# heracles-ec/heracles

Hardware: AMD Instinct MI355X
Metric: map->Cl pairs/sec + mixing-matrix build sec, nside=4096 lmax=6144 (higher is better)
Workload: dtype f64

## Files before the change

heracles_amd/csrc/hx_ring_fft.hip:

```cpp
#include <algorithm>
#include <type_traits>

#include "hx_sht_common.h"


namespace hx {
__global__ __launch_bounds__(512) void k_init_bhat(PlanDev P, const int *__restrict__ rp_list,
                                                   double2 *__restrict__ bhat)
{
    extern __shared__ double2 buf[];
    const int rp = rp_list[blockIdx.x];
    const int n = P.nsub[rp];
    const int M = fft_size_for(n);
    for (int j = threadIdx.x; j < lds_fft_slots(M); j += blockDim.x) buf[j] = make_double2(0.0, 0.0);
    __syncthreads();
    for (int j = threadIdx.x; j < n; j += blockDim.x) {
        double2 c = expipi((double)chirp_num(j, n) / (double)n);
        buf[lds_slot(j)] = c;
        if (j) buf[lds_slot(M - j)] = c;
    }
    __syncthreads();
    lds_fft_dif(buf, M, P.tw, P.twN);
    double2 *out = bhat + P.bhat_off[rp];
    for (int e = threadIdx.x; e < M; e += blockDim.x) out[M >= 16 ? (e & 15) * (M >> 4) + (e >> 4) : e] = buf[lds_slot(e)];
}

__host__ __device__ inline int ring_ph_hi(int M) { return (4 * M) / 64 + 1; }
constexpr int RING_NTMAX = 512;
constexpr int RING_FB = 8;

template <int MODE, bool WSYM = false>
__global__ __launch_bounds__(RING_NTMAX) void k_ring_subdft(PlanDev P, const RingDesc *__restrict__ desc, int nrings, int nb, int Mclass,
                                                            const double *__restrict__ maps,
                                                            const double *__restrict__ pixw,
                                                            const double2 *__restrict__ zin,
                                                            double2 *__restrict__ Y, double *__restrict__ pixout = nullptr,
                                                            const double *__restrict__ ref = nullptr)
{
    extern __shared__ double2 buf[];
    __shared__ double2 tw_hi[TW_HI_MAX], tw_lo[64];
    double2 *ph_hi = buf + lds_fft_slots(Mclass), *ph_lo = ph_hi + ring_ph_hi(Mclass);
    const int nt = blockDim.x;
    const int nitems = ((nrings + 7) >> 3) * nb * 32;
    const TwFactored twf = load_tw_factored(tw_hi, tw_lo, P.tw, P.twN);
    int tid = threadIdx.x;
    auto ring_of = [&](int item) __attribute__((always_inline)) { return ((item >> 5) / nb) * 8 + (item & 7); };
    RingDesc cur = RingDesc{0, 0, 0, 1, 0};
    if ((int)blockIdx.x < nitems && ring_of(blockIdx.x) < nrings) cur = desc[ring_of(blockIdx.x)];
    for (int item = blockIdx.x; item < nitems; item += gridDim.x) {
        const int r = (item >> 3) & 3, set = item >> 5;
        const int ring = ring_of(item), c = set % nb;
        const int itn = item + gridDim.x, ringn = itn < nitems ? ring_of(itn) : nrings;
        const bool nextv = ringn < nrings;
        if (ring >= nrings) {
            if (nextv) cur = desc[ringn];
            continue;
        }
        const int n = cur.n;
        const long long sN = cur.sN, sS = cur.sS;
        const int M = fft_size_for(n), MP = lds_fft_slots(M);
        const bool blu = M != n;
        const int p = ilog2(M);
        const double2 *bh = P.bhat + cur.bhat_off;
        const double inv = 1.0 / M, inv4n = 0.25 / (double)n;
        asm volatile("; item" : "+v"(tid));
        const bool haveS = sS >= 0, odd = r & 1, pw = MODE == 0 && !WSYM && pixw != nullptr;
        constexpr bool wsym = MODE == 0 && WSYM;
        const double sg = (r & 2) ? -1.0 : 1.0;
        const double *mpN = maps + (long long)c * P.npix + sN, *mpS = maps + (long long)c * P.npix + (haveS ? sS : sN);
        const double *pwN = pixw + sN, *pwS = pixw + (haveS ? sS : sN);
        const double2 *zp = zin + (long long)c * P.ny + sN;
        double2 z[RING_FB][4];
        struct __attribute__((aligned(8))) Pair { double x, y; };
        Pair wsy[RING_FB / 2];
        auto load_batch_t = [&](auto WIDEC, int u0) __attribute__((always_inline)) {
            constexpr bool WIDE = decltype(WIDEC)::value;
#pragma unroll
            for (int u = 0; u < RING_FB; u += 2) {
                const int j = 2 * (tid + ((u0 + u) >> 1) * nt);
                const bool tail = WIDE && j == n - 1;
                const int jj = tail ? n - 2 : (j + 1 < n ? j : 0);
                wsy[u >> 1] = Pair{1.0, 1.0};
                if (MODE == 0 && wsym && WIDE) wsy[u >> 1] = *reinterpret_cast<const Pair *>(pwN + jj);
#pragma unroll
                for (int q = 0; q < 4; ++q) {
                    const int i = jj + q * n;
                    if (MODE == 0) {
                        Pair fn, fs;
                        if (WIDE) {
                            fn = *reinterpret_cast<const Pair *>(mpN + i);
                            fs = *reinterpret_cast<const Pair *>(mpS + i);
                            if (!wsym && pw) {
                                const Pair wn = *reinterpret_cast<const Pair *>(pwN + i), ws = *reinterpret_cast<const Pair *>(pwS + i);
                                fn.x *= wn.x; fn.y *= wn.y; fs.x *= ws.x; fs.y *= ws.y;
                            }
// ... 16 lines not shown
        auto load_batch = [&](int u0) __attribute__((always_inline)) {
            if (n >= 2) load_batch_t(std::true_type{}, u0);
            else load_batch_t(std::false_type{}, u0);
        };
        auto finish_batch = [&](int u0) __attribute__((always_inline)) {
            if (MODE != 0 || n < 2) return;
#pragma unroll
            for (int u = 0; u < RING_FB; u += 2) {
                const int j = 2 * (tid + ((u0 + u) >> 1) * nt);
                const bool tail = j == n - 1;
                const Pair w = wsy[u >> 1];
#pragma unroll
                for (int q = 0; q < 4; ++q) {
                    const double2 rn = z[u][q], rs = z[u + 1][q];
                    const double nx = wsym ? rn.x * w.x : rn.x, ny = wsym ? rn.y * w.y : rn.y;
                    const double sx = wsym ? rs.x * w.x : rs.x, sy = wsym ? rs.y * w.y : rs.y;
                    z[u][q] = make_double2(tail ? ny : nx, haveS ? (tail ? sy : sx) : 0.0);
                    z[u + 1][q] = make_double2(ny, haveS ? sy : 0.0);
                }
            }
        };
        load_batch(0);
        int4 nd0 = make_int4(0, 0, 0, 0), nd1 = nd0;
        if (nextv) {
            const int4 *dp = reinterpret_cast<const int4 *>(desc + ringn) + (tid >> 30);
            nd0 = dp[0];
            nd1 = dp[1];
        }
        auto lds_barrier = []() __attribute__((always_inline)) {
            __builtin_amdgcn_s_waitcnt(0xc07f);
            __builtin_amdgcn_s_barrier();
        };
        lds_barrier();
        for (int a = tid; a <= (4 * n) >> 6; a += nt) ph_hi[a] = expipi(-(double)(a << 6) / (2.0 * n));
        if (tid < 64) ph_lo[tid] = expipi(-(double)tid / (2.0 * n));
        lds_barrier();
        auto phase = [&](unsigned q) __attribute__((always_inline)) {
            return cmul(ph_hi[q >> 6], ph_lo[q & 63]);
        };
        {
            for (int u0 = 0;;) {
                finish_batch(u0);
#pragma unroll
                for (int u = 0; u < RING_FB; ++u) {
                    const int j = 2 * (tid + ((u0 + u) >> 1) * nt) + (u & 1);
                    const double2 e0 = odd ? csub(z[u][0], z[u][2]) : cadd(z[u][0], z[u][2]);
                    const double2 e1 = odd ? mul_mi(csub(z[u][1], z[u][3])) : cadd(z[u][1], z[u][3]);
                    const double2 t = make_double2(fma(sg, e1.x, e0.x), fma(sg, e1.y, e0.y));
                    const unsigned jc = j < n ? j : 0;
                    const unsigned qn = blu ? mod_by_inv(jc * (unsigned)r + 2u * jc * jc, 4u * (unsigned)n, inv4n) : jc * (unsigned)r;
                    buf[j < n ? lds_slot(j) : MP - 1] = cmul(t, phase(qn));
                }
                u0 += RING_FB;
                if (u0 * nt >= n) break;
                load_batch(u0);
            }
            if (blu)
                for (int j = n + tid; j < M; j += nt) buf[lds_slot(j)] = make_double2(0.0, 0.0);
        }
        __syncthreads();
        if (nextv) {
            auto sc = [](int v) __attribute__((always_inline)) { return __builtin_amdgcn_readfirstlane(v); };
            cur.sN = ((long long)sc(nd0.y) << 32) | (unsigned)sc(nd0.x);
            cur.sS = ((long long)sc(nd0.w) << 32) | (unsigned)sc(nd0.z);
            cur.bhat_off = ((long long)sc(nd1.y) << 32) | (unsigned)sc(nd1.x);
            cur.n = sc(nd1.z);
            cur.rp = sc(nd1.w);
        }
        double2 *out = Y + (long long)c * P.ny + sN + (long long)r * n;
        double *pxN = nullptr, *pxS = nullptr;
        const double *rfN = nullptr, *rfS = nullptr;
        if (MODE == 1 && pixout) {
            pxN = pixout + (long long)c * P.npix + sN + r;
            pxS = pixout + (long long)c * P.npix + (haveS ? sS : sN) + r;
            if (ref) { rfN = ref + (long long)c * P.npix + sN + r; rfS = ref + (long long)c * P.npix + (haveS ? sS : sN) + r; }
        }
        const int kdrop0 = MODE == 0 ? (P.lmax - r) / 4 + 1 : n, kdrop1 = (4 * n - P.lmax - r + 3) / 4;
        auto emit = [&](int k, double2 v) __attribute__((always_inline)) {
            if (MODE == 0 && k >= kdrop0 && k < kdrop1) return;
            if (MODE == 1 && pxN) {
                double fn = v.x, fs = -v.y;
                if (rfN) { fn = rfN[4 * k] - fn; fs = rfS[4 * k] - fs; }
                pxN[4 * k] = fn;
                if (haveS) pxS[4 * k] = fs;
            } else {
                out[k] = v;
            }
        };
        if (!blu) {
            lds_fft_dif(buf, M, twf, P.twN);
            for (int k = tid; k < n; k += nt) emit(k, buf[lds_slot(bitrev(k, p))]);
            continue;
        }
        if (M >= 16) {
            double2 bq[16];
            const int nbf = M >> 4;
#pragma unroll
            for (int j = 0; j < 16; ++j) bq[j] = bh[j * nbf + (tid < nbf ? tid : 0)];
            lds_fft_dif(buf, M, twf, P.twN, tid, nt, true);
#pragma unroll 1
            for (int i = tid; i < nbf; i += nt) {
                double2 x[16];
#pragma unroll
                for (int j = 0; j < 16; ++j) x[j] = buf[lds_slot(16 * i) + j];
                dif_regs<4>(x);
#pragma unroll
                for (int j = 0; j < 16; ++j) {
                    x[j] = cmul(x[j], bq[j]);
                }
                if (i + nt < nbf) {
#pragma unroll
                    for (int j = 0; j < 16; ++j) bq[j] = bh[j * nbf + i + nt];
                }
                dit_inv_regs<4>(x);
#pragma unroll
                for (int j = 0; j < 16; ++j) buf[lds_slot(16 * i) + j] = x[j];
            }
            __syncthreads();
            lds_fft_dit_inv(buf, M, twf, P.twN, tid, nt, true);
        } else {
            lds_fft_dif(buf, M, twf, P.twN, tid, nt);
            for (int j = tid; j < M; j += nt) buf[lds_slot(j)] = cmul(buf[lds_slot(j)], bh[j]);
            __syncthreads();
            lds_fft_dit_inv(buf, M, twf, P.twN, tid, nt);
        }
        for (int k = tid; k < n; k += nt)
            emit(k, cscale(cmul(buf[lds_slot(k)], phase(2u * mod_by_inv((unsigned)k * (unsigned)k, 2u * (unsigned)n, 2.0 * inv4n))), inv));
    }
}

template <int MODE, bool WSYM = false>
__global__ __launch_bounds__(RING_NTMAX) void k_ring_pairfft(PlanDev P, const RingDesc *__restrict__ desc, int nrings, int nb, int M,
                                                             const double *__restrict__ maps, const double *__restrict__ pixw,
                                                             const double2 *__restrict__ zin, double2 *__restrict__ Y,
                                                             double *__restrict__ pixout = nullptr, const double *__restrict__ ref = nullptr)
{
    extern __shared__ double2 buf[];
    __shared__ double2 tw_hi[TW_HI_MAX], tw_lo[64];
    const int MP = lds_fft_slots(M), n = M, p = ilog2(M);
    double2 *ph_hi = buf + 2 * MP, *ph_lo = ph_hi + ring_ph_hi(M);
    const int nt = blockDim.x, nh = nt >> 1;
    const int nitems = ((nrings + 7) >> 3) * nb * 16;
    const TwFactored twf = load_tw_factored(tw_hi, tw_lo, P.tw, P.twN);
    int tid = threadIdx.x;
    for (int a = tid; a <= (4 * n) >> 6; a += nt) ph_hi[a] = expipi(-(double)(a << 6) / (2.0 * n));
    if (tid < 64) ph_lo[tid] = expipi(-(double)tid / (2.0 * n));
    __syncthreads();
    auto phase = [&](unsigned q) __attribute__((always_inline)) { return cmul(ph_hi[q >> 6], ph_lo[q & 63]); };
    auto ring_of = [&](int item) __attribute__((always_inline)) { return ((item >> 4) / nb) * 8 + (item & 7); };
    auto comp_of = [&](int item) __attribute__((always_inline)) { return (item >> 4) % nb; };
    RingDesc cur = RingDesc{0, 0, 0, 1, 0};
    if ((int)blockIdx.x < nitems && ring_of(blockIdx.x) < nrings) cur = desc[ring_of(blockIdx.x)];
    struct __attribute__((aligned(8))) Pair { double x, y; };
    double2 z[RING_FB][4];
    Pair wsy[RING_FB / 2];
    const bool pw = MODE == 0 && !WSYM && pixw != nullptr;
    constexpr bool wsym = MODE == 0 && WSYM;
    auto request = [&](auto U0C, const RingDesc &d, int c) __attribute__((always_inline)) {
        constexpr int U0 = decltype(U0C)::value;
        const bool hS = d.sS >= 0;
// ... 80 lines not shown
            request(H0{}, cur, comp_of(itn));
            have_half = true;
        }
        const int half = tid >= nh ? 1 : 0, gt = tid - half * nh;
        double2 *bh = buf + half * MP;
        lds_fft_dif(bh, M, twf, P.twN, gt, nh);
        const int r = rpair + 2 * half;
        if (MODE == 1 && pixout) {
            double *pxN = pixout + (long long)c * P.npix + sN + r, *pxS = pixout + (long long)c * P.npix + (haveS ? sS : sN) + r;
            if (ref) {
                const double *rfN = ref + (long long)c * P.npix + sN + r, *rfS = ref + (long long)c * P.npix + (haveS ? sS : sN) + r;
                for (int k = gt; k < n; k += nh) {
                    const double2 v = bh[lds_slot(bitrev(k, p))];
                    pxN[4 * k] = rfN[4 * k] - v.x;
                    if (haveS) pxS[4 * k] = rfS[4 * k] + v.y;
                }
            } else {
                for (int k = gt; k < n; k += nh) {
                    const double2 v = bh[lds_slot(bitrev(k, p))];
                    pxN[4 * k] = v.x;
                    if (haveS) pxS[4 * k] = -v.y;
                }
            }
        } else {
            double2 *out = Y + (long long)c * P.ny + sN + (long long)r * n;
            const int kdrop0 = MODE == 0 ? (P.lmax - r) / 4 + 1 : n, kdrop1 = (4 * n - P.lmax - r + 3) / 4;
            for (int k = gt; k < n; k += nh)
                if (k < kdrop0 || k >= kdrop1) *(out + k) = bh[lds_slot(bitrev(k, p))];
        }
        }
    }
}

constexpr int SPLIT_JMAX = 16;

__global__ __launch_bounds__(512) void k_init_bhat_split(PlanDev P, const int *__restrict__ rp_list, int C,
                                                          double2 *__restrict__ bhat)
{
    extern __shared__ double2 buf[];
    const int rp = rp_list[blockIdx.x];
    const int n = P.nsub[rp], M = 2 * C;
    double2 *out = bhat + P.bhat_off[rp];
    auto b_at = [&](int j) {
        const int jj = j < n ? j : (M - j < n ? M - j : -1);
        return jj < 0 ? make_double2(0.0, 0.0) : expipi((double)chirp_num(jj, n) / (double)n);
    };
    for (int half = 0; half < 2; ++half) {
        __syncthreads();
        for (int j = threadIdx.x; j < C; j += blockDim.x) {
            const double2 b0 = b_at(j), b1 = b_at(j + C);
            buf[lds_slot(j)] = half == 0 ? cadd(b0, b1) : cmul(csub(b0, b1), P.tw[j]);
        }
        __syncthreads();
        lds_fft_dif(buf, C, P.tw, P.twN);
        for (int j = threadIdx.x; j < C; j += blockDim.x) out[half * C + j] = buf[lds_slot(j)];
    }
}

template <int MODE>
__global__ __launch_bounds__(512) void k_ring_subdft_split(PlanDev P, const int *__restrict__ rp_list, int C,
                                                            const double *__restrict__ maps, const double *__restrict__ pixw,
                                                            const double2 *__restrict__ zin, double2 *__restrict__ Y,
                                                            double *__restrict__ pixout = nullptr, const double *__restrict__ ref = nullptr)
{
    extern __shared__ double2 buf[];
    const int rp = rp_list[blockIdx.y];
// ... 94 lines not shown
__global__ __launch_bounds__(256) void k_pixw_symmetry(PlanDev P, const double *__restrict__ pixw, int *__restrict__ flag)
{
    const int rp = blockIdx.x, n = P.nsub[rp];
    const long long sN = P.startN[rp], sS = P.startS[rp];
    bool ok = true;
    for (int j = threadIdx.x; j < n; j += blockDim.x) {
        const double w = pixw[sN + j];
#pragma unroll
        for (int q = 1; q < 4; ++q) ok = ok && pixw[sN + j + (long long)q * n] == w;
        if (sS >= 0) {
#pragma unroll
            for (int q = 0; q < 4; ++q) ok = ok && pixw[sS + j + (long long)q * n] == w;
        }
    }
    if (!ok) *flag = 0;
}

}

using namespace hx;

static int g_lds_fft_cap = 8192;
extern "C" int hx_set_max_lds_fft(int points)
{
    if (points < 16 || points > 8192 || (points & (points - 1))) return fail(HX_ERR_ARG, "hx_set_max_lds_fft: a power of two in [16, 8192]");
    g_lds_fft_cap = points;
    return HX_OK;
}

static size_t ring_class_lds(int M, bool pair) { return ((pair ? 2 : 1) * (size_t)lds_fft_slots(M) + ring_ph_hi(M) + 64) * sizeof(double2); }

static bool ring_class_is_pair(int n, int M, int cap) { return M == n && M >= 16 && M <= cap && ring_class_lds(M, true) + 4096 <= 160 * 1024; }

int hx::ring_fft_plan_init(hx_plan *pl, const std::vector<int> &nsub, const std::vector<long long> &sN, const std::vector<long long> &sS)
{
    const int cap = g_lds_fft_cap;
    std::map<std::pair<int, int>, std::vector<int>> byM;
    bool plain_beyond_cap = false;
    for (int rp = pl->nrp - 1; rp >= 0; --rp) {
        const int M = fft_size_for(nsub[rp]);
        byM[{M, ring_class_is_pair(nsub[rp], M, cap) ? -1 : 0}].push_back(rp);
        plain_beyond_cap = plain_beyond_cap || (M > cap && M == nsub[rp]);
    }
    const int maxM = byM.rbegin()->first.first;
    if (maxM > 2 * cap || plain_beyond_cap) return fail(HX_ERR_UNSUPPORTED, "hx_plan_create: nside=%d needs an in-LDS FFT of %d points (limit %d, %d for Bluestein rings); unsupported", pl->nside, maxM, cap, 2 * cap);
    pl->fft_cap = cap;
    pl->lds_fft = (size_t)lds_fft_slots(std::min(maxM, cap)) * sizeof(double2);
    for (auto it = byM.rbegin(); it != byM.rend(); ++it) {
        pl->fft_classes.push_back({it->first.first, (int)pl->h_fft_rp_list.size(), (int)it->second.size(), it->first.second});
        pl->h_fft_rp_list.insert(pl->h_fft_rp_list.end(), it->second.begin(), it->second.end());
    }
    HX_TRY(upload(pl->fft_rp_list, pl->h_fft_rp_list));
    std::vector<long long> boff(pl->nrp, -1);
    std::vector<int> blu_list, blu_split;
    long long btot = 0;
    std::map<int, long long> off_of_n;
    for (int rp = 0; rp < pl->nrp; ++rp) {
        int n = nsub[rp], M = fft_size_for(n);
        if (M == n) continue;
        auto it = off_of_n.find(n);
        if (it == off_of_n.end()) {
            it = off_of_n.emplace(n, btot).first;
            btot += M;
            (M > cap ? blu_split : blu_list).push_back(rp);
        }
        boff[rp] = it->second;
    }
    HX_TRY(upload(pl->bhat_off, boff));
    std::vector<RingDesc> desc;
    for (int rp : pl->h_fft_rp_list) desc.push_back(RingDesc{sN[rp], sS[rp], boff[rp], nsub[rp], rp});
    HX_TRY(upload(pl->fft_desc, desc));
    HX_TRY(pl->bhat.alloc(sizeof(double2) * std::max<long long>(btot, 1)));
    const void *const init_kernels[] = {(const void *)k_init_bhat, (const void *)k_init_bhat_split};
    const void *const ring_kernels[] = {(const void *)k_ring_subdft<0, false>,  (const void *)k_ring_subdft<0, true>,  (const void *)k_ring_subdft<1, false>,
                                        (const void *)k_ring_pairfft<0, false>, (const void *)k_ring_pairfft<0, true>, (const void *)k_ring_pairfft<1, false>,
                                        (const void *)k_ring_subdft_split<0>,   (const void *)k_ring_subdft_split<1>};
    for (const void *k : init_kernels) (void)hipFuncSetAttribute(k, hipFuncAttributeMaxDynamicSharedMemorySize, 160 * 1024);
    for (const void *k : ring_kernels) (void)hipFuncSetAttribute(k, hipFuncAttributeMaxDynamicSharedMemorySize, 156 * 1024);
    HX_HIP(hipGetLastError());
    hipStream_t st = rt().stream;
    if (!blu_list.empty()) {
        DevBuf d_list;
        HX_TRY(upload(d_list, blu_list));
        hipLaunchKernelGGL(k_init_bhat, dim3((unsigned)blu_list.size()), dim3(512), pl->lds_fft, st, pl->dev(),
                           d_list.as<int>(), pl->bhat.as<double2>());
        (void)hipStreamSynchronize(st);
    }
    if (!blu_split.empty()) {
        DevBuf d_list;
        HX_TRY(upload(d_list, blu_split));
        hipLaunchKernelGGL(k_init_bhat_split, dim3((unsigned)blu_split.size()), dim3(std::min(512, std::max(64, cap / 16))), (size_t)lds_fft_slots(cap) * sizeof(double2), st,
                           pl->dev(), d_list.as<int>(), cap, pl->bhat.as<double2>());
        (void)hipStreamSynchronize(st);
    }
    return HX_OK;
}

struct RingIO { const double *maps, *pixw; const double2 *zin; double2 *Y; double *pixout; const double *ref; };

template <auto KERNEL>
static void launch_ring_class(hx_plan *pl, const hx_plan::FftClass &c, int nb, const RingIO &io)
{
    const int k = c.big < 0 ? 2 : 1;
    const int threads = std::min(RING_NTMAX, k * std::max(64, c.M / 16));
    const size_t lds = ring_class_lds(c.M, k == 2);
    const int per_cu = (int)std::max<size_t>(1, std::min<size_t>(512 / threads, (160 * 1024) / (lds + 3 * 1024 + 256)));
    const long long items = ((long long)c.count + 7) / 8 * nb * (32 / k);
    const unsigned groups = (unsigned)std::min<long long>(items, (long long)rt().cus * per_cu);
    hipLaunchKernelGGL(KERNEL, dim3(groups), dim3(threads), lds, rt().stream, pl->dev(), pl->fft_desc.as<RingDesc>() + c.first, c.count, nb, c.M, io.maps, io.pixw, io.zin, io.Y, io.pixout, io.ref);
}

template <int MODE, bool WSYM>
static int launch_subdft_classes(hx_plan *pl, int nb, const RingIO &io, int rp_lo = 0, int rp_hi = 0x7fffffff)
{
    for (const auto &cls : pl->fft_classes) {
        hx_plan::FftClass c = cls;
        if (rp_lo > 0 || rp_hi < pl->nrp) {
            const int *b = pl->h_fft_rp_list.data() + cls.first, *e = b + cls.count;
            const int *x = std::lower_bound(b, e, rp_hi, [](int rp, int lim) { return rp >= lim; });
            const int *y = std::lower_bound(b, e, rp_lo, [](int rp, int lim) { return rp >= lim; });
            c.first = cls.first + (int)(x - b);
            c.count = (int)(y - x);
            if (c.count <= 0) continue;
        }
        if (c.big < 0)
            launch_ring_class<k_ring_pairfft<MODE, WSYM>>(pl, c, nb, io);
        else if (c.M > pl->fft_cap) {
            const int C = pl->fft_cap, threads = std::min(512, std::max(64, C / SPLIT_JMAX));
            hipLaunchKernelGGL(k_ring_subdft_split<MODE>, dim3(1, c.count, nb), dim3(threads), (size_t)lds_fft_slots(C) * sizeof(double2), rt().stream,
                               pl->dev(), pl->fft_rp_list.as<int>() + c.first, C, io.maps, io.pixw, io.zin, io.Y, io.pixout, io.ref);
        } else
            launch_ring_class<k_ring_subdft<MODE, WSYM>>(pl, c, nb, io);
    }
    HX_HIP(hipGetLastError());
    return HX_OK;
}

int hx::launch_ring_subdft_maps(hx_plan *pl, int nb, const double *d_maps, const double *d_pw, double2 *Y, int rp_lo, int rp_hi)
{
    ProfScope ps("ring_fft");
    if (d_pw && pl->pw_checked != d_pw) HX_TRY(classify_pixel_weights(pl, d_pw));
    const RingIO io = {d_maps, d_pw, nullptr, Y, nullptr, nullptr};
    return d_pw && pl->pw_mode == 2 ? launch_subdft_classes<0, true>(pl, nb, io, rp_lo, rp_hi) : launch_subdft_classes<0, false>(pl, nb, io, rp_lo, rp_hi);
}

int hx::launch_ring_subdft_spectra(hx_plan *pl, int nc, const double2 *zin, double *pixout, const double *ref)
{
    return launch_subdft_classes<1, false>(pl, nc, RingIO{nullptr, nullptr, zin, nullptr, pixout, ref});
}

int hx::classify_pixel_weights(hx_plan *pl, const double *d_pw)
{
    pl->pw_checked = d_pw;
    pl->pw_mode = 0;
    if (!d_pw || pl->nside < 1) return HX_OK;
    HX_TRY(pl->pw_sym.alloc(sizeof(int)));
    HX_HIP(hipMemsetAsync(pl->pw_sym.p, 1, sizeof(int), rt().stream));
    hipLaunchKernelGGL(k_pixw_symmetry, dim3(pl->nrp), dim3(256), 0, rt().stream, pl->dev(), d_pw, pl->pw_sym.as<int>());
    int flag = 0;
    HX_HIP(hipMemcpyAsync(&flag, pl->pw_sym.p, sizeof(int), hipMemcpyDeviceToHost, rt().stream));
    HX_HIP(hipStreamSynchronize(rt().stream));
    pl->pw_mode = flag != 0 ? 2 : 1;
    return HX_OK;
}
// ... 1 lines not shown
```

heracles_amd/csrc/hx_fft_core.h:

```cpp
#pragma once
#ifdef __HIPCC__
#include <hip/hip_runtime.h>
#define HX_HD __host__ __device__ __forceinline__
#else
#include <cmath>
#define HX_HD inline
struct double2 {
    double x, y;
};
#endif

namespace hxfft {

HX_HD double2 mk(double a, double b)
{
    double2 r;
    r.x = a;
    r.y = b;
    return r;
}
HX_HD double2 cadd(double2 a, double2 b) { return mk(a.x + b.x, a.y + b.y); }
HX_HD double2 csub(double2 a, double2 b) { return mk(a.x - b.x, a.y - b.y); }
HX_HD double2 cmul(double2 a, double2 b) { return mk(a.x * b.x - a.y * b.y, a.x * b.y + a.y * b.x); }
HX_HD double2 cmulc(double2 a, double2 b)
// ... 132 lines not shown
{
    constexpr int R = 1 << K;
    const int t = i & (h - 1), p = ((i - t) << K) + t;
    double2 x[R];
#ifdef __HIPCC__
#pragma unroll
#endif
    for (int j = 0; j < R; ++j) x[j] = buf[lds_slot(p + j * h)];
    dif_regs<K>(x);
    if (h > 1 && t) apply_tw_powers<K, false>(x, tw[t * (twN / (R * h))]);
#ifdef __HIPCC__
#pragma unroll
#endif
    for (int j = 0; j < R; ++j) buf[lds_slot(p + j * h)] = x[j];
}
template <int K, class TW>
HX_HD void dit_inv_pass_butterfly(double2 *buf, int i, int h, TW tw, int twN)
{
    constexpr int R = 1 << K;
    const int t = i & (h - 1), p = ((i - t) << K) + t;
    double2 x[R];
#ifdef __HIPCC__
#pragma unroll
#endif
    for (int j = 0; j < R; ++j) x[j] = buf[lds_slot(p + j * h)];
    if (h > 1 && t) apply_tw_powers<K, true>(x, tw[t * (twN / (R * h))]);
    dit_inv_regs<K>(x);
#ifdef __HIPCC__
#pragma unroll
#endif
    for (int j = 0; j < R; ++j) buf[lds_slot(p + j * h)] = x[j];
}

HX_HD int fft_sched_np(int p) { return p <= 0 ? 0 : (p - (p < 4 ? p : 4) + 3) / 4 + 1; }
HX_HD int fft_sched_k(int p, int a)
{
    const int last = p < 4 ? p : 4, rest = p - last, nfront = (rest + 3) / 4;
    return a < nfront ? rest / nfront + (a < rest % nfront ? 1 : 0) : last;
}

HX_HD double2 dif4_combine(double2 z0, double2 z1, double2 z2, double2 z3, int r)
{
    switch (r & 3) {
    case 0: return cadd(cadd(z0, z1), cadd(z2, z3));
    case 1: return cadd(csub(z0, z2), mul_mi(csub(z1, z3)));
    case 2: return cadd(csub(z0, z1), csub(z2, z3));
    default: return cadd(csub(z0, z2), mul_pi(csub(z1, z3)));
    }
}

HX_HD unsigned mod_by_inv(unsigned x, unsigned d, double inv)
{
    const int q = (int)((double)x * inv);
    int r = (int)x - q * (int)d;
    if (r < 0) r += (int)d;
    if (r >= (int)d) r -= (int)d;
    return (unsigned)r;
}

HX_HD unsigned load_phase_num(unsigned j, unsigned r, unsigned n, bool bluestein)
{
    unsigned long long q = (unsigned long long)j * r;
    if (bluestein) q += 2ull * j * j;
    return (unsigned)(q % (4ull * n));
}

// ... 7 lines not shown
```

heracles_amd/csrc/hx_sht_common.h:

```cpp
#pragma once
#include <map>
#include <vector>

#include "hx_common.h"
#include "hx_fft_core.h"

namespace hx {

typedef double double4_t __attribute__((ext_vector_type(4)));

constexpr int LBLK = 32;
constexpr int NCOL = 16;
constexpr int TABLE_PAD = 512;
constexpr int NGMAX = 2;
constexpr int RBLK = 32;
constexpr double SC_BIG = 0x1p+300, SC_SMALL = 0x1p-300;
constexpr int SPIN_ANY = -1;

struct LegTask {
    int m;
    int rb0;
    int nrb;
    int pad;
    long long pout;
};

struct MTasks {
    int first, count;
};

struct alignas(16) RingDesc {
    long long sN, sS, bhat_off;
    int n, rp;
};
// ... 174 lines not shown

template <class TW>
__device__ __forceinline__ void lds_fft_pass_dif(double2 *buf, int M, int K, int h, int gt, int gn, TW tw, int twN)
{
    switch (K) {
    case 4:
_Pragma("unroll 1")
        for (int i = gt; i < (M >> 4); i += gn) dif_pass_butterfly<4>(buf, i, h, tw, twN); break;
    case 3:
_Pragma("unroll 1")
        for (int i = gt; i < (M >> 3); i += gn) dif_pass_butterfly<3>(buf, i, h, tw, twN); break;
    case 2:
_Pragma("unroll 1")
        for (int i = gt; i < (M >> 2); i += gn) dif_pass_butterfly<2>(buf, i, h, tw, twN); break;
    default: for (int i = gt; i < (M >> 1); i += gn) dif_pass_butterfly<1>(buf, i, h, tw, twN); break;
    }
}
template <class TW>
__device__ __forceinline__ void lds_fft_pass_dit_inv(double2 *buf, int M, int K, int h, int gt, int gn, TW tw, int twN)
{
    switch (K) {
    case 4:
_Pragma("unroll 1")
        for (int i = gt; i < (M >> 4); i += gn) dit_inv_pass_butterfly<4>(buf, i, h, tw, twN); break;
    case 3:
_Pragma("unroll 1")
        for (int i = gt; i < (M >> 3); i += gn) dit_inv_pass_butterfly<3>(buf, i, h, tw, twN); break;
    case 2:
_Pragma("unroll 1")
        for (int i = gt; i < (M >> 2); i += gn) dit_inv_pass_butterfly<2>(buf, i, h, tw, twN); break;
    default: for (int i = gt; i < (M >> 1); i += gn) dit_inv_pass_butterfly<1>(buf, i, h, tw, twN); break;
    }
}
template <class TW>
__device__ __forceinline__ void lds_fft_dif(double2 *buf, int M, TW tw, int twN, int gt, int gn, bool skip_last = false)
{
    const int p = ilog2(M), np = fft_sched_np(p);
    int h = M;
    for (int a = 0; a < np - (skip_last ? 1 : 0); ++a) {
        const int K = fft_sched_k(p, a);
        h >>= K;
        lds_fft_pass_dif(buf, M, K, h, gt, gn, tw, twN);
        __syncthreads();
    }
}
template <class TW>
__device__ __forceinline__ void lds_fft_dit_inv(double2 *buf, int M, TW tw, int twN, int gt, int gn, bool skip_first = false)
{
    const int p = ilog2(M), np = fft_sched_np(p);
    int h = 1;
    for (int a = np - 1; a >= 0; --a) {
        const int K = fft_sched_k(p, a);
        if (!(skip_first && a == np - 1)) {
            lds_fft_pass_dit_inv(buf, M, K, h, gt, gn, tw, twN);
            __syncthreads();
        }
        h <<= K;
    }
}
template <class TW>
__device__ __forceinline__ void lds_fft_dif(double2 *buf, int M, TW tw, int twN) { lds_fft_dif(buf, M, tw, twN, (int)threadIdx.x, (int)blockDim.x); }
template <class TW>
__device__ __forceinline__ void lds_fft_dit_inv(double2 *buf, int M, TW tw, int twN) { lds_fft_dit_inv(buf, M, tw, twN, (int)threadIdx.x, (int)blockDim.x); }

constexpr int TW_HI_MAX = 128;
__device__ inline TwFactored load_tw_factored(double2 *hi, double2 *lo, const double2 *__restrict__ tw, int twN)
{
    for (int i = threadIdx.x; i < (twN >= 128 ? twN / 128 : 1); i += blockDim.x) hi[i] = tw[i * 64];
    for (int i = threadIdx.x; i < 64; i += blockDim.x) lo[i] = tw[i];
    TwFactored f;
    f.hi = hi;
    f.lo = lo;
    return f;
}

#endif

template <class T>
inline int upload(DevBuf &b, const std::vector<T> &v)
{
    HX_TRY(b.alloc(sizeof(T) * (v.size() > 0 ? v.size() : 1)));
    if (!v.empty()) HX_HIP(hipMemcpy(b.p, v.data(), sizeof(T) * v.size(), hipMemcpyHostToDevice));
    return HX_OK;
}

}

// ... 99 lines not shown
```

Measured before the change: 427.8.

## Add paired Bluestein ring kernel processing two sub-DFTs per item

Adds a k_ring_blupair kernel for Bluestein rings (M != n) in analysis mode. Each work item loads the ring data once and computes the pre-twiddled inputs for two residue classes r and r+2 together. The second one is stashed in registers and swapped into LDS inside the convolution step. Per-ring phase tables are precomputed into the bhat buffer at plan init instead of being rebuilt per item, and the Bluestein convolution is factored into a shared helper. This cuts map reads and per-item setup in half, at the cost of more registers, a larger bhat allocation and more complex item indexing.

```diff
diff --git a/heracles_amd/csrc/hx_ring_fft.hip b/heracles_amd/csrc/hx_ring_fft.hip
--- a/heracles_amd/csrc/hx_ring_fft.hip
+++ b/heracles_amd/csrc/hx_ring_fft.hip
@@ -25,9 +25,71 @@
     for (int e = threadIdx.x; e < M; e += blockDim.x) out[M >= 16 ? (e & 15) * (M >> 4) + (e >> 4) : e] = buf[lds_slot(e)];
 }
 
+__global__ __launch_bounds__(512) void k_init_phase_tables(PlanDev P, const int *__restrict__ rp_list, double2 *__restrict__ bhat)
+{
+    const int rp = rp_list[blockIdx.x];
+    const int n = P.nsub[rp], nhi = ((4 * n) >> 6) + 1;
+    double2 *out = bhat + P.bhat_off[rp] + fft_size_for(n);
+    for (int a = threadIdx.x; a < nhi + 64; a += blockDim.x) out[a] = expipi(-(double)(a < nhi ? a << 6 : a - nhi) / (2.0 * n));
+}
+
 __host__ __device__ inline int ring_ph_hi(int M) { return (4 * M) / 64 + 1; }
 constexpr int RING_NTMAX = 512;
 constexpr int RING_FB = 8;
+
+template <int NKEEP = 0, class TW>
+__device__ __forceinline__ void ring_bluestein_conv(double2 *buf, int M, const double2 *__restrict__ bh, TW twf, int twN, int tid, int nt,
+                                                    double2 *keep = nullptr)
+{
+    double2 bq[16];
+    const int nbf = M >> 4;
+#pragma unroll
+    for (int j = 0; j < 16; ++j) bq[j] = bh[j * nbf + (tid < nbf ? tid : 0)];
+    lds_fft_dif(buf, M, twf, twN, tid, nt, true);
+    if (NKEEP > 0) {
+        if (tid < nbf) {
+            double2 x[16];
+            double2 *own = buf + lds_slot(16 * tid);
+#pragma unroll
+            for (int j = 0; j < 16; ++j) x[j] = own[j];
+#pragma unroll
+            for (int u = 0; u < NKEEP; ++u) own[u] = keep[u];
+            asm volatile("" ::: "memory");
+            dif_regs<4>(x);
+#pragma unroll
+            for (int j = 0; j < 16; ++j) x[j] = cmul(x[j], bq[j]);
+            dit_inv_regs<4>(x);
+            asm volatile("" ::: "memory");
+#pragma unroll
+            for (int u = 0; u < NKEEP; ++u) keep[u] = own[u];
+#pragma unroll
+            for (int j = 0; j < 16; ++j) own[j] = x[j];
+        } else {
+#pragma unroll
+            for (int u = 0; u < NKEEP; ++u) keep[u] = make_double2(0.0, 0.0);
+        }
+    } else
+#pragma unroll 1
+    for (int i = tid; i < nbf; i += nt) {
+        double2 x[16];
+#pragma unroll
+        for (int j = 0; j < 16; ++j) x[j] = buf[lds_slot(16 * i) + j];
+        dif_regs<4>(x);
+#pragma unroll
+        for (int j = 0; j < 16; ++j) {
+            x[j] = cmul(x[j], bq[j]);
+        }
+        if (i + nt < nbf) {
+#pragma unroll
+            for (int j = 0; j < 16; ++j) bq[j] = bh[j * nbf + i + nt];
+        }
+        dit_inv_regs<4>(x);
+#pragma unroll
+        for (int j = 0; j < 16; ++j) buf[lds_slot(16 * i) + j] = x[j];
+    }
+    __syncthreads();
+    lds_fft_dit_inv(buf, M, twf, twN, tid, nt, true);
+}
 
 template <int MODE, bool WSYM = false>
 __global__ __launch_bounds__(RING_NTMAX) void k_ring_subdft(PlanDev P, const RingDesc *__restrict__ desc, int nrings, int nb, int Mclass,
@@ -204,31 +266,7 @@
             continue;
         }
         if (M >= 16) {
-            double2 bq[16];
-            const int nbf = M >> 4;
-#pragma unroll
-            for (int j = 0; j < 16; ++j) bq[j] = bh[j * nbf + (tid < nbf ? tid : 0)];
-            lds_fft_dif(buf, M, twf, P.twN, tid, nt, true);
-#pragma unroll 1
-            for (int i = tid; i < nbf; i += nt) {
-                double2 x[16];
-#pragma unroll
-                for (int j = 0; j < 16; ++j) x[j] = buf[lds_slot(16 * i) + j];
-                dif_regs<4>(x);
-#pragma unroll
-                for (int j = 0; j < 16; ++j) {
-                    x[j] = cmul(x[j], bq[j]);
-                }
-                if (i + nt < nbf) {
-#pragma unroll
-                    for (int j = 0; j < 16; ++j) bq[j] = bh[j * nbf + i + nt];
-                }
-                dit_inv_regs<4>(x);
-#pragma unroll
-                for (int j = 0; j < 16; ++j) buf[lds_slot(16 * i) + j] = x[j];
-            }
-            __syncthreads();
-            lds_fft_dit_inv(buf, M, twf, P.twN, tid, nt, true);
+            ring_bluestein_conv(buf, M, bh, twf, P.twN, tid, nt);
         } else {
             lds_fft_dif(buf, M, twf, P.twN, tid, nt);
             for (int j = tid; j < M; j += nt) buf[lds_slot(j)] = cmul(buf[lds_slot(j)], bh[j]);
@@ -383,6 +421,164 @@
     }
 }
 
+template <bool WSYM>
+__global__ __launch_bounds__(RING_NTMAX) void k_ring_blupair(PlanDev P, const RingDesc *__restrict__ desc, int nrings, int nb, int Mclass,
+                                                             const double *__restrict__ maps, const double *__restrict__ pixw,
+                                                             const double2 *__restrict__, double2 *__restrict__ Y,
+                                                             double *__restrict__ = nullptr, const double *__restrict__ = nullptr)
+{
+    extern __shared__ double2 buf[];
+    __shared__ double2 tw_hi[TW_HI_MAX], tw_lo[64];
+    double2 *ph_hi = buf + lds_fft_slots(Mclass);
+    const int nt = blockDim.x;
+    const int nitems = ((nrings + 7) >> 3) * nb * 16;
+    const TwFactored twf = load_tw_factored(tw_hi, tw_lo, P.tw, P.twN);
+    int tid = threadIdx.x;
+    auto ring_of = [&](int item) __attribute__((always_inline)) { return ((item >> 4) / nb) * 8 + (item & 7); };
+    RingDesc cur = RingDesc{0, 0, 0, 1, 0};
+    if ((int)blockIdx.x < nitems && ring_of(blockIdx.x) < nrings) cur = desc[ring_of(blockIdx.x)];
+    for (int item = blockIdx.x; item < nitems; item += gridDim.x) {
+        const int rpair = (item >> 3) & 1;
+        const int ring = ring_of(item), c = (item >> 4) % nb;
+        const int itn = item + gridDim.x, ringn = itn < nitems ? ring_of(itn) : nrings;
+        const bool nextv = ringn < nrings;
+        if (ring >= nrings) {
+            if (nextv) cur = desc[ringn];
+            continue;
+        }
+        const int n = cur.n;
+        const long long sN = cur.sN, sS = cur.sS;
+        const int M = fft_size_for(n), MP = lds_fft_slots(M);
+        const double2 *bh = P.bhat + cur.bhat_off;
+        const double inv4n = 0.25 / (double)n;
+        asm volatile("; item" : "+v"(tid));
+        const bool haveS = sS >= 0, pw = !WSYM && pixw != nullptr;
+        const int nf = M >> 4;
+        auto fill_thread = [&]() __attribute__((always_inline)) {
+            int t = tid;
+            asm volatile("; j" : "+v"(t));
+            return t < nf ? t : 1 << 20;
+        };
+        const double *mpN = maps + (long long)c * P.npix + sN, *mpS = maps + (long long)c * P.npix + (haveS ? sS : sN);
+        const double *pwN = pixw + sN, *pwS = pixw + (haveS ? sS : sN);
+        const int nhi = ((4 * n) >> 6) + 1, ntab = nhi + 64;
+        double2 *ph_lo = ph_hi + nhi;
+        const double2 tab0 = bh[M + (tid < ntab ? tid : 0)], tab1 = bh[M + (tid + nt < ntab ? tid + nt : 0)];
+        struct __attribute__((aligned(8))) Pair { double x, y; };
+        double2 z[RING_FB][4];
+        Pair wsy[RING_FB / 2];
+        auto pair_at = [](const double *base, int i) __attribute__((always_inline)) {
+            return *reinterpret_cast<const Pair *>(reinterpret_cast<const char *>(base) + (unsigned)(i * 8));
+        };
+        int tf = fill_thread();
+#pragma unroll
+        for (int u = 0; u < RING_FB; u += 2) {
+            const int j = 2 * (tf + (u >> 1) * nf);
+            const int jj = j == n - 1 ? n - 2 : (j + 1 < n ? j : 0);
+            wsy[u >> 1] = Pair{1.0, 1.0};
+            if (WSYM) wsy[u >> 1] = pair_at(pwN, jj);
+#pragma unroll
+            for (int q = 0; q < 4; ++q) {
+                const int i = jj + q * n;
+                Pair fn = pair_at(mpN, i), fs = pair_at(mpS, i);
+                if (!WSYM && pw) {
+                    const Pair wn = pair_at(pwN, i), ws = pair_at(pwS, i);
+                    fn.x *= wn.x; fn.y *= wn.y; fs.x *= ws.x; fs.y *= ws.y;
+                }
+                z[u][q] = make_double2(fn.x, fn.y);
+                z[u + 1][q] = make_double2(fs.x, fs.y);
+            }
+        }
+        int4 nd0 = make_int4(0, 0, 0, 0), nd1 = nd0;
+        if (nextv) {
+            const int4 *dp = reinterpret_cast<const int4 *>(desc + ringn) + (tid >> 30);
+            nd0 = dp[0];
+            nd1 = dp[1];
+        }
+        auto lds_barrier = []() __attribute__((always_inline)) {
+            __builtin_amdgcn_s_waitcnt(0xc07f);
+            __builtin_amdgcn_s_barrier();
+        };
+        lds_barrier();
+        if (tid < ntab) ph_hi[tid] = tab0;
+        if (tid + nt < ntab) ph_hi[tid + nt] = tab1;
+        lds_barrier();
+        auto cmulf = [](double2 a, double2 b) __attribute__((always_inline)) {
+            return make_double2(__builtin_fma(a.x, b.x, -(a.y * b.y)), __builtin_fma(a.x, b.y, a.y * b.x));
+        };
+        auto phase = [&](unsigned q) __attribute__((always_inline)) {
+            const double2 h = ph_hi[q >> 6], l = ph_lo[q & 63];
+            return make_double2(__builtin_fma(h.x, l.x, -(h.y * l.y)), __builtin_fma(h.y, l.x, h.x * l.y));
+        };
+        double2 stash[RING_FB];
+        tf = fill_thread();
+        {
+#pragma clang fp contract(off)
+#pragma unroll
+        for (int u = 0; u < RING_FB; u += 2) {
+            const int j = 2 * (tf + (u >> 1) * nf);
+            const bool tail = j == n - 1;
+            const Pair w = wsy[u >> 1];
+#pragma unroll
+            for (int q = 0; q < 4; ++q) {
+                const double2 rn = z[u][q], rs = z[u + 1][q];
+                const double nx = WSYM ? rn.x * w.x : rn.x, ny = WSYM ? rn.y * w.y : rn.y;
+                const double sx = WSYM ? rs.x * w.x : rs.x, sy = WSYM ? rs.y * w.y : rs.y;
+                z[u][q] = make_double2(tail ? ny : nx, haveS ? (tail ? sy : sx) : 0.0);
+                z[u + 1][q] = make_double2(ny, haveS ? sy : 0.0);
+            }
+        }
+#pragma unroll
+        for (int u = 0; u < RING_FB; ++u) {
+            const int j = 2 * (tf + (u >> 1) * nf) + (u & 1);
+            const double2 e0 = rpair ? csub(z[u][0], z[u][2]) : cadd(z[u][0], z[u][2]);
+            const double2 e1 = rpair ? mul_mi(csub(z[u][1], z[u][3])) : cadd(z[u][1], z[u][3]);
+            const double2 t0 = cadd(e0, e1), t2 = csub(e0, e1);
+            const unsigned jc = j < n ? j : 0;
+            const unsigned q0 = mod_by_inv(jc * (unsigned)rpair + 2u * jc * jc, 4u * (unsigned)n, inv4n);
+            const unsigned q2s = q0 + 2u * jc, q2 = q2s >= 4u * (unsigned)n ? q2s - 4u * (unsigned)n : q2s;
+            buf[j < n ? lds_slot(j) : MP - 1] = cmulf(t0, phase(q0));
+            stash[u] = cmulf(t2, phase(q2));
+        }
+        }
+        for (int j = n + tid; j < M; j += nt) buf[lds_slot(j)] = make_double2(0.0, 0.0);
+        __syncthreads();
+        if (nextv) {
+            auto sc = [](int v) __attribute__((always_inline)) { return __builtin_amdgcn_readfirstlane(v); };
+            cur.sN = ((long long)sc(nd0.y) << 32) | (unsigned)sc(nd0.x);
+            cur.sS = ((long long)sc(nd0.w) << 32) | (unsigned)sc(nd0.z);
+            cur.bhat_off = ((long long)sc(nd1.y) << 32) | (unsigned)sc(nd1.x);
+            cur.n = sc(nd1.z);
+            cur.rp = sc(nd1.w);
+        }
+#pragma unroll 1
+        for (int half = 0; half < 2; ++half) {
+            const int r = rpair + 2 * half;
+            int th = tid, ne = n, Me = M;
+            asm volatile("; half" : "+v"(th), "+s"(ne), "+s"(Me));
+            if (half) {
+                lds_barrier();
+                const int ts = fill_thread();
+#pragma unroll
+                for (int u = 0; u < RING_FB; ++u) {
+                    const int j = 2 * (ts + (u >> 1) * nf) + (u & 1);
+                    buf[j < n ? lds_slot(j) : MP - 1] = stash[u];
+                }
+                for (int j = ne + th; j < Me; j += nt) buf[lds_slot(j)] = make_double2(0.0, 0.0);
+                lds_barrier();
+            }
+            ring_bluestein_conv<RING_FB>(buf, M, bh, twf, P.twN, th, nt, stash);
+            double2 *out = Y + (long long)c * P.ny + sN + (long long)r * n;
+            const int kdrop0 = (P.lmax - r) / 4 + 1, kdrop1 = (4 * n - P.lmax - r + 3) / 4;
+            const double inv2n = 2.0 * (0.25 / (double)ne), invM = 1.0 / Me;
+            for (int k = th; k < n; k += nt) {
+                if (k >= kdrop0 && k < kdrop1) continue;
+                out[k] = cscale(cmulf(buf[lds_slot(k)], phase(2u * mod_by_inv((unsigned)k * (unsigned)k, 2u * (unsigned)n, inv2n))), invM);
+            }
+        }
+    }
+}
+
 constexpr int SPLIT_JMAX = 16;
 
 __global__ __launch_bounds__(512) void k_init_bhat_split(PlanDev P, const int *__restrict__ rp_list, int C,
@@ -543,6 +739,8 @@
 
 static bool ring_class_is_pair(int n, int M, int cap) { return M == n && M >= 16 && M <= cap && ring_class_lds(M, true) + 4096 <= 160 * 1024; }
 
+static bool ring_class_is_blupair(int n, int M, int cap) { return M != n && M >= 16 && M <= cap; }
+
 int hx::ring_fft_plan_init(hx_plan *pl, const std::vector<int> &nsub, const std::vector<long long> &sN, const std::vector<long long> &sS)
 {
     const int cap = g_lds_fft_cap;
@@ -550,7 +748,7 @@
     bool plain_beyond_cap = false;
     for (int rp = pl->nrp - 1; rp >= 0; --rp) {
         const int M = fft_size_for(nsub[rp]);
-        byM[{M, ring_class_is_pair(nsub[rp], M, cap) ? -1 : 0}].push_back(rp);
+        byM[{M, ring_class_is_pair(nsub[rp], M, cap) ? -1 : ring_class_is_blupair(nsub[rp], M, cap) ? 1 : 0}].push_back(rp);
         plain_beyond_cap = plain_beyond_cap || (M > cap && M == nsub[rp]);
     }
     const int maxM = byM.rbegin()->first.first;
@@ -572,7 +770,7 @@
         auto it = off_of_n.find(n);
         if (it == off_of_n.end()) {
             it = off_of_n.emplace(n, btot).first;
-            btot += M;
+            btot += M + (M > cap ? 0 : ring_ph_hi(M) + 64);
             (M > cap ? blu_split : blu_list).push_back(rp);
         }
         boff[rp] = it->second;
@@ -585,6 +783,7 @@
     const void *const init_kernels[] = {(const void *)k_init_bhat, (const void *)k_init_bhat_split};
     const void *const ring_kernels[] = {(const void *)k_ring_subdft<0, false>,  (const void *)k_ring_subdft<0, true>,  (const void *)k_ring_subdft<1, false>,
                                         (const void *)k_ring_pairfft<0, false>, (const void *)k_ring_pairfft<0, true>, (const void *)k_ring_pairfft<1, false>,
+                                        (const void *)k_ring_blupair<false>,    (const void *)k_ring_blupair<true>,
                                         (const void *)k_ring_subdft_split<0>,   (const void *)k_ring_subdft_split<1>};
     for (const void *k : init_kernels) (void)hipFuncSetAttribute(k, hipFuncAttributeMaxDynamicSharedMemorySize, 160 * 1024);
     for (const void *k : ring_kernels) (void)hipFuncSetAttribute(k, hipFuncAttributeMaxDynamicSharedMemorySize, 156 * 1024);
@@ -595,6 +794,7 @@
         HX_TRY(upload(d_list, blu_list));
         hipLaunchKernelGGL(k_init_bhat, dim3((unsigned)blu_list.size()), dim3(512), pl->lds_fft, st, pl->dev(),
                            d_list.as<int>(), pl->bhat.as<double2>());
+        hipLaunchKernelGGL(k_init_phase_tables, dim3((unsigned)blu_list.size()), dim3(512), 0, st, pl->dev(), d_list.as<int>(), pl->bhat.as<double2>());
         (void)hipStreamSynchronize(st);
     }
     if (!blu_split.empty()) {
@@ -612,9 +812,10 @@
 template <auto KERNEL>
 static void launch_ring_class(hx_plan *pl, const hx_plan::FftClass &c, int nb, const RingIO &io)
 {
-    const int k = c.big < 0 ? 2 : 1;
-    const int threads = std::min(RING_NTMAX, k * std::max(64, c.M / 16));
-    const size_t lds = ring_class_lds(c.M, k == 2);
+    const bool blupair = KERNEL == k_ring_blupair<false> || KERNEL == k_ring_blupair<true>;
+    const int side = c.big < 0 ? 2 : 1, k = blupair ? 2 : side;
+    const int threads = std::min(RING_NTMAX, side * std::max(64, c.M / 16));
+    const size_t lds = ring_class_lds(c.M, side == 2);
     const int per_cu = (int)std::max<size_t>(1, std::min<size_t>(512 / threads, (160 * 1024) / (lds + 3 * 1024 + 256)));
     const long long items = ((long long)c.count + 7) / 8 * nb * (32 / k);
     const unsigned groups = (unsigned)std::min<long long>(items, (long long)rt().cus * per_cu);
@@ -640,7 +841,9 @@
             const int C = pl->fft_cap, threads = std::min(512, std::max(64, C / SPLIT_JMAX));
             hipLaunchKernelGGL(k_ring_subdft_split<MODE>, dim3(1, c.count, nb), dim3(threads), (size_t)lds_fft_slots(C) * sizeof(double2), rt().stream,
                                pl->dev(), pl->fft_rp_list.as<int>() + c.first, C, io.maps, io.pixw, io.zin, io.Y, io.pixout, io.ref);
-        } else
+        } else if (MODE == 0 && c.big > 0)
+            launch_ring_class<k_ring_blupair<WSYM>>(pl, c, nb, io);
+        else
             launch_ring_class<k_ring_subdft<MODE, WSYM>>(pl, c, nb, io);
     }
     HX_HIP(hipGetLastError());
```

New measurement: 431.6 (median of 6 runs). No clear change (+0.9%).

## Prune zero-padded Bluestein FFT passes and cache ring phase tables

Applied to the files above, without the earlier changes.

Adds input-pruned first DIF passes and output-pruned last inverse DIT passes for Bluestein ring FFTs, where only the first n of M entries are nonzero or needed. When log2(M) mod 4 equals 1, it also folds the top radix-2 stage into the load and emit steps, so the LDS FFT runs at half size. Zero-fill of the padding is limited to a short tail, and the phase tables are rebuilt only when the ring length changes. This cuts FFT butterfly work and LDS traffic, at the cost of heavy template instantiation that can raise register pressure and code size, and the pruned butterflies need a per-butterfly live-count branch.

```diff
diff --git a/heracles_amd/csrc/hx_fft_core.h b/heracles_amd/csrc/hx_fft_core.h
--- a/heracles_amd/csrc/hx_fft_core.h
+++ b/heracles_amd/csrc/hx_fft_core.h
@@ -188,6 +188,111 @@
     for (int j = 0; j < R; ++j) buf[lds_slot(p + j * h)] = x[j];
 }
 
+constexpr int FFT_LIVE_TAIL = 64;
+
+HX_HD int fft_live_count(int K, int h, int n, int t0)
+{
+    const int half = 1 << (K - 1), L = n > t0 ? (n - t0 + h - 1) >> (31 - __builtin_clz((unsigned)h)) : 0;
+    return L < half ? L : half;
+}
+
+template <int K, int L>
+HX_HD void dif_regs_live(double2 *x)
+{
+    constexpr int R = 1 << K;
+    static_assert(L >= 0 && L <= R, "live inputs of a radix-2^K butterfly");
+    unsigned live = (1u << L) - 1u;
+#ifdef __HIPCC__
+#pragma unroll
+#endif
+    for (int s = 0; s < K; ++s) {
+        const int half = R >> (s + 1);
+#ifdef __HIPCC__
+#pragma unroll
+#endif
+        for (int b = 0; b < R; b += 2 * half)
+#ifdef __HIPCC__
+#pragma unroll
+#endif
+            for (int jj = 0; jj < half; ++jj) {
+                const int a = b + jj, c = a + half, k = jj * (8 / half);
+                const bool la = (live >> a) & 1u, lc = (live >> c) & 1u;
+                const double2 u = x[a], v = x[c];
+                if (la && lc) {
+                    x[a] = cadd(u, v);
+                    x[c] = rot16(csub(u, v), k);
+                } else if (la) {
+                    x[c] = rot16(u, k);
+                } else if (lc) {
+                    x[a] = v;
+                    x[c] = rot16(mk(-v.x, -v.y), k);
+                }
+                if (la || lc) live |= (1u << a) | (1u << c);
+            }
+    }
+#ifdef __HIPCC__
+#pragma unroll
+#endif
+    for (int j = 0; j < R; ++j)
+        if (!((live >> j) & 1u)) x[j] = mk(0.0, 0.0);
+}
+
+template <int K, int L, class TW>
+HX_HD void dif_pass_butterfly_live(double2 *buf, int i, int h, TW tw, int twN)
+{
+    constexpr int R = 1 << K;
+    const int t = i & (h - 1), p = ((i - t) << K) + t;
+    double2 x[R];
+#ifdef __HIPCC__
+#pragma unroll
+#endif
+    for (int j = 0; j < R; ++j) x[j] = j < L ? buf[lds_slot(p + j * h)] : mk(0.0, 0.0);
+    dif_regs_live<K, L>(x);
+    if (L > 0 && h > 1 && t) apply_tw_powers<K, false>(x, tw[t * (twN / (R * h))]);
+#ifdef __HIPCC__
+#pragma unroll
+#endif
+    for (int j = 0; j < R; ++j) buf[lds_slot(p + j * h)] = x[j];
+}
+template <int K, int L, class TW>
+HX_HD void dit_inv_pass_butterfly_keep(double2 *buf, int i, int h, TW tw, int twN)
+{
+    constexpr int R = 1 << K;
+    if (L == 0) return;
+    const int t = i & (h - 1), p = ((i - t) << K) + t;
+    double2 x[R];
+#ifdef __HIPCC__
+#pragma unroll
+#endif
+    for (int j = 0; j < R; ++j) x[j] = buf[lds_slot(p + j * h)];
+    if (h > 1 && t) apply_tw_powers<K, true>(x, tw[t * (twN / (R * h))]);
+    dit_inv_regs<K>(x);
+#ifdef __HIPCC__
+#pragma unroll
+#endif
+    for (int j = 0; j < L; ++j) buf[lds_slot(p + j * h)] = x[j];
+}
+template <int K, int L = (1 << K) / 2, class TW>
+HX_HD void dif_pass_butterfly_live_n(double2 *buf, int i, int h, int Lrt, TW tw, int twN)
+{
+    if constexpr (L <= (1 << K) / 4) {
+        dif_pass_butterfly_live<K, L>(buf, i, h, tw, twN);
+    } else {
+        if (Lrt >= L) dif_pass_butterfly_live<K, L>(buf, i, h, tw, twN);
+        else dif_pass_butterfly_live_n<K, L - 1>(buf, i, h, Lrt, tw, twN);
+    }
+}
+template <int K, int L = (1 << K) / 2, class TW>
+HX_HD void dit_inv_pass_butterfly_keep_n(double2 *buf, int i, int h, int Lrt, TW tw, int twN)
+{
+    if constexpr (L <= (1 << K) / 4) {
+        dit_inv_pass_butterfly_keep<K, L>(buf, i, h, tw, twN);
+    } else {
+        if (Lrt >= L) dit_inv_pass_butterfly_keep<K, L>(buf, i, h, tw, twN);
+        else dit_inv_pass_butterfly_keep_n<K, L - 1>(buf, i, h, Lrt, tw, twN);
+    }
+}
+
 HX_HD int fft_sched_np(int p) { return p <= 0 ? 0 : (p - (p < 4 ? p : 4) + 3) / 4 + 1; }
 HX_HD int fft_sched_k(int p, int a)
 {
diff --git a/heracles_amd/csrc/hx_ring_fft.hip b/heracles_amd/csrc/hx_ring_fft.hip
--- a/heracles_amd/csrc/hx_ring_fft.hip
+++ b/heracles_amd/csrc/hx_ring_fft.hip
@@ -47,6 +47,7 @@
     auto ring_of = [&](int item) __attribute__((always_inline)) { return ((item >> 5) / nb) * 8 + (item & 7); };
     RingDesc cur = RingDesc{0, 0, 0, 1, 0};
     if ((int)blockIdx.x < nitems && ring_of(blockIdx.x) < nrings) cur = desc[ring_of(blockIdx.x)];
+    int tab_n = 0;
     for (int item = blockIdx.x; item < nitems; item += gridDim.x) {
         const int r = (item >> 3) & 3, set = item >> 5;
         const int ring = ring_of(item), c = set % nb;
@@ -61,6 +62,7 @@
         const int M = fft_size_for(n), MP = lds_fft_slots(M);
         const bool blu = M != n;
         const int p = ilog2(M);
+        const int pre = blu && M >= 32 && (p & 3) == 1 ? 1 : 0, twsh = ilog2(P.twN) - p;
         const double2 *bh = P.bhat + cur.bhat_off;
         const double inv = 1.0 / M, inv4n = 0.25 / (double)n;
         asm volatile("; item" : "+v"(tid));
@@ -143,9 +145,12 @@
             __builtin_amdgcn_s_barrier();
         };
         lds_barrier();
-        for (int a = tid; a <= (4 * n) >> 6; a += nt) ph_hi[a] = expipi(-(double)(a << 6) / (2.0 * n));
-        if (tid < 64) ph_lo[tid] = expipi(-(double)tid / (2.0 * n));
-        lds_barrier();
+        if (n != tab_n) {
+            for (int a = tid; a <= (4 * n) >> 6; a += nt) ph_hi[a] = expipi(-(double)(a << 6) / (2.0 * n));
+            if (tid < 64) ph_lo[tid] = expipi(-(double)tid / (2.0 * n));
+            lds_barrier();
+            tab_n = n;
+        }
         auto phase = [&](unsigned q) __attribute__((always_inline)) {
             return cmul(ph_hi[q >> 6], ph_lo[q & 63]);
         };
@@ -166,8 +171,15 @@
                 if (u0 * nt >= n) break;
                 load_batch(u0);
             }
-            if (blu)
-                for (int j = n + tid; j < M; j += nt) buf[lds_slot(j)] = make_double2(0.0, 0.0);
+            if (pre) {
+                for (int j = 2 * tid; j < n; j += 2 * nt) {
+                    buf[lds_slot(j + (M >> 1))] = cmul(buf[lds_slot(j)], twf[j << twsh]);
+                    if (j + 1 < n) buf[lds_slot(j + 1 + (M >> 1))] = cmul(buf[lds_slot(j + 1)], twf[(j + 1) << twsh]);
+                }
+                for (int j = n + tid; j < (M >> 1); j += nt) buf[lds_slot(j)] = buf[lds_slot(j + (M >> 1))] = make_double2(0.0, 0.0);
+            } else if (blu) {
+                for (int j = n + tid; j < min(M, n + FFT_LIVE_TAIL); j += nt) buf[lds_slot(j)] = make_double2(0.0, 0.0);
+            }
         }
         __syncthreads();
         if (nextv) {
@@ -208,7 +220,7 @@
             const int nbf = M >> 4;
 #pragma unroll
             for (int j = 0; j < 16; ++j) bq[j] = bh[j * nbf + (tid < nbf ? tid : 0)];
-            lds_fft_dif(buf, M, twf, P.twN, tid, nt, true);
+            lds_fft_dif(buf, M, twf, P.twN, tid, nt, true, n, pre);
 #pragma unroll 1
             for (int i = tid; i < nbf; i += nt) {
                 double2 x[16];
@@ -228,15 +240,18 @@
                 for (int j = 0; j < 16; ++j) buf[lds_slot(16 * i) + j] = x[j];
             }
             __syncthreads();
-            lds_fft_dit_inv(buf, M, twf, P.twN, tid, nt, true);
+            lds_fft_dit_inv(buf, M, twf, P.twN, tid, nt, true, n, pre);
         } else {
             lds_fft_dif(buf, M, twf, P.twN, tid, nt);
             for (int j = tid; j < M; j += nt) buf[lds_slot(j)] = cmul(buf[lds_slot(j)], bh[j]);
             __syncthreads();
             lds_fft_dit_inv(buf, M, twf, P.twN, tid, nt);
         }
-        for (int k = tid; k < n; k += nt)
-            emit(k, cscale(cmul(buf[lds_slot(k)], phase(2u * mod_by_inv((unsigned)k * (unsigned)k, 2u * (unsigned)n, 2.0 * inv4n))), inv));
+        for (int k = tid; k < n; k += nt) {
+            double2 y = buf[lds_slot(k)];
+            if (pre) y = cadd(y, cmulc(buf[lds_slot(k + (M >> 1))], twf[k << twsh]));
+            emit(k, cscale(cmul(y, phase(2u * mod_by_inv((unsigned)k * (unsigned)k, 2u * (unsigned)n, 2.0 * inv4n))), inv));
+        }
     }
 }
 
diff --git a/heracles_amd/csrc/hx_sht_common.h b/heracles_amd/csrc/hx_sht_common.h
--- a/heracles_amd/csrc/hx_sht_common.h
+++ b/heracles_amd/csrc/hx_sht_common.h
@@ -1,5 +1,6 @@
 #pragma once
 #include <map>
+#include <type_traits>
 #include <vector>
 
 #include "hx_common.h"
@@ -240,27 +241,48 @@
     default: for (int i = gt; i < (M >> 1); i += gn) dit_inv_pass_butterfly<1>(buf, i, h, tw, twN); break;
     }
 }
-template <class TW>
-__device__ __forceinline__ void lds_fft_dif(double2 *buf, int M, TW tw, int twN, int gt, int gn, bool skip_last = false)
-{
-    const int p = ilog2(M), np = fft_sched_np(p);
-    int h = M;
+template <bool FORWARD, class TW>
+__device__ __forceinline__ void lds_fft_pass_pruned(double2 *buf, int M, int K, int h, int gt, int gn, int n, TW tw, int twN)
+{
+    auto run = [&](auto KC) __attribute__((always_inline)) {
+        constexpr int KK = decltype(KC)::value;
+_Pragma("unroll 1")
+        for (int i = gt; i < (M >> KK); i += gn) {
+            const int L = fft_live_count(KK, h, n, __builtin_amdgcn_readfirstlane(i));
+            if (FORWARD) dif_pass_butterfly_live_n<KK>(buf, i, h, L, tw, twN);
+            else dit_inv_pass_butterfly_keep_n<KK>(buf, i, h, L, tw, twN);
+        }
+    };
+    switch (K) {
+    case 4: run(std::integral_constant<int, 4>{}); break;
+    case 3: run(std::integral_constant<int, 3>{}); break;
+    case 2: run(std::integral_constant<int, 2>{}); break;
+    default: run(std::integral_constant<int, 1>{}); break;
+    }
+}
+template <class TW>
+__device__ __forceinline__ void lds_fft_dif(double2 *buf, int M, TW tw, int twN, int gt, int gn, bool skip_last = false, int nlive = 0, int pre = 0)
+{
+    const int p = ilog2(M) - pre, np = fft_sched_np(p);
+    int h = M >> pre;
     for (int a = 0; a < np - (skip_last ? 1 : 0); ++a) {
         const int K = fft_sched_k(p, a);
         h >>= K;
-        lds_fft_pass_dif(buf, M, K, h, gt, gn, tw, twN);
+        if (a == 0 && nlive > 0 && pre == 0 && h > 1) lds_fft_pass_pruned<true>(buf, M, K, h, gt, gn, nlive, tw, twN);
+        else lds_fft_pass_dif(buf, M, K, h, gt, gn, tw, twN);
         __syncthreads();
     }
 }
 template <class TW>
-__device__ __forceinline__ void lds_fft_dit_inv(double2 *buf, int M, TW tw, int twN, int gt, int gn, bool skip_first = false)
-{
-    const int p = ilog2(M), np = fft_sched_np(p);
+__device__ __forceinline__ void lds_fft_dit_inv(double2 *buf, int M, TW tw, int twN, int gt, int gn, bool skip_first = false, int nkeep = 0, int pre = 0)
+{
+    const int p = ilog2(M) - pre, np = fft_sched_np(p);
     int h = 1;
     for (int a = np - 1; a >= 0; --a) {
         const int K = fft_sched_k(p, a);
         if (!(skip_first && a == np - 1)) {
-            lds_fft_pass_dit_inv(buf, M, K, h, gt, gn, tw, twN);
+            if (a == 0 && nkeep > 0 && pre == 0 && h > 1) lds_fft_pass_pruned<false>(buf, M, K, h, gt, gn, nkeep, tw, twN);
+            else lds_fft_pass_dit_inv(buf, M, K, h, gt, gn, tw, twN);
             __syncthreads();
         }
         h <<= K;
```

After: 425.2 before, 427.0 after, median of 6. Within noise of the previous version (+0.4%).
